# microsoft/NOTSOFAR1-Challenge

Measured on AMD Instinct MI355X. Metric: CSS real-time-factor (sep. audio sec/wall sec) on 7-ch 16 kHz, higher is better.
Workload: dtype f32 (float32 operands on v_mfma_f32_32x32x2_f32 in every Linear layer, attention product and transform: the reference's own operand precision; MVDR covariance / solve f64)

## Files before the change

include/css_mi355.h:

```cpp
#ifndef CSS_MI355_H
#define CSS_MI355_H

#include <stddef.h>
#include <stdint.h>

#ifdef __cplusplus
extern "C" {
#endif
#if defined(__GNUC__) || defined(__clang__)
#pragma GCC visibility push(default)
#endif

typedef struct css_ctx* css_handle_t;

typedef enum css_status {
    CSS_OK = 0,
    CSS_ERR_INVALID_ARG = -1,
    CSS_ERR_HIP = -2,
    CSS_ERR_ZERO_WEIGHT = -3,
    CSS_ERR_MASK_FLOOR = -4,
    CSS_ERR_SHAPE = -5,
    CSS_ERR_STATE = -6,
    CSS_ERR_NO_DEVICE = -7,
    CSS_ERR_WEIGHT_WINDOW = -8,
// ... 136 lines not shown
int css_run_enqueue(css_handle_t h, const float* pcm_host, int64_t n_samples, int32_t n_ch, const CssRunCfg* cfg,
                    float* wav_host, int64_t cap);
int css_set_queue_group(css_handle_t h, int max_sessions);
int css_wait(css_handle_t h);
int css_wait_sessions(css_handle_t h, int64_t n);
int css_run_device(css_handle_t h, const float* pcm_dev, int64_t n_samples, int32_t n_ch, const CssRunCfg* cfg,
                   float* wav_dev, int64_t wav_capacity_per_stream);
int css_run_pcm16(css_handle_t h, const int16_t* const* planes_host, int64_t n_samples, int32_t n_ch, const CssRunCfg* cfg,
                  int16_t* wav_pcm16_host, int64_t wav_capacity_per_stream, float* peaks_host);
int css_run_enqueue_pcm16(css_handle_t h, const int16_t* const* planes_host, int64_t n_samples, int32_t n_ch, const CssRunCfg* cfg,
                          int16_t* wav_pcm16_host, int64_t wav_capacity_per_stream, float* peaks_host);
int css_get_timings(css_handle_t h, CssTimings* out);
int css_set_profile(css_handle_t h, int enable);
typedef struct CssKernelStat { char name[32]; float ms; int32_t launches; } CssKernelStat;
int css_get_kernel_stats(css_handle_t h, CssKernelStat* out, int32_t cap, int32_t* count);
enum css_linear_mode { CSS_LINEAR_SPLIT_F16 = 0, CSS_LINEAR_EXACT_F32 = 1 };
int css_set_linear_mode(css_handle_t h, int mode);
int css_get_linear_mode(css_handle_t h);
int css_set_range_fallback(css_handle_t h, int enable);
int css_range_status(css_handle_t h, int64_t* fallbacks, int32_t* last_hit);
int css_check_range(css_handle_t h);
int css_linear_host(css_handle_t h, const float* x, const float* w, const float* bias, int32_t M, int32_t N, int32_t K,
                    int32_t kernel, int32_t layout, float* y);
int css_get_plan(css_handle_t h, CssPlan* out);

int css_begin(css_handle_t h, const float* pcm, int64_t n_samples, int32_t n_ch, const CssRunCfg* cfg, int pcm_is_device);
int css_begin_range(css_handle_t h, const float* pcm_host, int64_t n_samples, int32_t n_ch, const CssRunCfg* cfg,
                    int64_t s_lo, int64_t s_hi);
int css_upload_range(css_handle_t h, const float* pcm_host, int64_t s_lo, int64_t s_hi);
int css_stage_stft(css_handle_t h);
int css_stage_stft_range(css_handle_t h, int64_t t_lo, int64_t t_hi);
int css_stage_masknet(css_handle_t h, int64_t seg_lo, int64_t seg_hi);
int css_stage_mvdr(css_handle_t h, int64_t seg_lo, int64_t seg_hi);
int css_stage_pit_costs(css_handle_t h, int64_t b_lo, int64_t b_hi);
int css_stage_pit_scan(css_handle_t h);
int css_stage_stitch(css_handle_t h, int64_t t_lo, int64_t t_hi);
int css_stage_istft(css_handle_t h, int64_t t_lo, int64_t t_hi);
int css_stage_stitch_masks(css_handle_t h, int64_t t_lo, int64_t t_hi);
int css_stage_stitch_gate(css_handle_t h, int64_t t_lo, int64_t t_hi);
int css_stage_istft_partial(css_handle_t h, int64_t t_lo, int64_t t_hi, float* shard_dev, int64_t shard_ld);
int css_stage_synthesis(css_handle_t h, int64_t t_lo, int64_t t_hi);
int css_stage_seam_rows(css_handle_t h, int64_t t_lo, int64_t t_hi, float* rows_dev, int32_t write);
int css_stage_overlap_add(css_handle_t h, int64_t f_lo, int64_t f_hi, int64_t q_lo, int64_t q_hi, float* out_dev, int64_t out_ld,
                          int64_t out_q0);
int css_stage_join_shards(css_handle_t h, const float* gathered_dev, int32_t world, int64_t shard_ld, const int64_t* t_lo,
                          const int64_t* t_hi, float* out_dev, int64_t out_ld);
// ... 66 lines not shown
```

notsofar1-challenge_amd/_lib.py:

```python
from __future__ import annotations

import ctypes as C
import os
from typing import Optional

import numpy as np

_HERE = os.path.dirname(os.path.abspath(__file__))
LIB_PATH = os.environ.get("CSS_MI355_LIBRARY") or os.path.join(_HERE, "libcss_mi355.so")


class CssLibraryError(RuntimeError):
    pass


class CssError(RuntimeError):
    def __init__(self, code: int, text: str):
        super().__init__(f"css_mi355 error {code}: {text}")
        self.code = code
        self.text = text


CSS_OK, CSS_ERR_INVALID_ARG, CSS_ERR_HIP, CSS_ERR_ZERO_WEIGHT, CSS_ERR_MASK_FLOOR = 0, -1, -2, -3, -4
CSS_ERR_SHAPE, CSS_ERR_STATE, CSS_ERR_NO_DEVICE, CSS_ERR_WEIGHT_WINDOW, CSS_ERR_RANGE = -5, -6, -7, -8, -9
# ... 80 lines not shown
    "css_set_tuning": (C.c_int, [_P, C.c_int, C.c_int]),
    "css_set_queue_group": (C.c_int, [_P, C.c_int]),
    "css_host_alloc": (C.c_int, [C.c_size_t, C.POINTER(_P)]),
    "css_host_free": (C.c_int, [_P]),
    "css_plan": (C.c_int, [C.POINTER(CssModelDesc), C.POINTER(CssRunCfg), C.c_int64, C.POINTER(CssPlan)]),
    "css_make_run_cfg": (C.c_int, [C.POINTER(CssModelDesc), C.POINTER(CssCfgSeconds), C.c_int32, C.POINTER(CssRunCfg), _FP, C.c_int64]),
    "css_pit_scan": (C.c_int, [_P, C.c_int64, C.c_int32, _P]),
    "css_run": (C.c_int, [_P, _P, C.c_int64, C.c_int32, C.POINTER(CssRunCfg), _P, C.c_int64]),
    "css_run_enqueue": (C.c_int, [_P, _P, C.c_int64, C.c_int32, C.POINTER(CssRunCfg), _P, C.c_int64]),
    "css_wait": (C.c_int, [_P]),
    "css_wait_sessions": (C.c_int, [_P, C.c_int64]),
    "css_run_device": (C.c_int, [_P, _P, C.c_int64, C.c_int32, C.POINTER(CssRunCfg), _P, C.c_int64]),
    "css_run_pcm16": (C.c_int, [_P, _P, C.c_int64, C.c_int32, C.POINTER(CssRunCfg), _P, C.c_int64, _P]),
    "css_run_enqueue_pcm16": (C.c_int, [_P, _P, C.c_int64, C.c_int32, C.POINTER(CssRunCfg), _P, C.c_int64, _P]),
    "css_get_timings": (C.c_int, [_P, C.POINTER(CssTimings)]),
    "css_set_profile": (C.c_int, [_P, C.c_int]),
    "css_get_kernel_stats": (C.c_int, [_P, _P, C.c_int32, C.POINTER(C.c_int32)]),
    "css_set_linear_mode": (C.c_int, [_P, C.c_int]),
    "css_get_linear_mode": (C.c_int, [_P]),
    "css_set_range_fallback": (C.c_int, [_P, C.c_int]),
    "css_range_status": (C.c_int, [_P, C.POINTER(C.c_int64), C.POINTER(C.c_int32)]),
    "css_check_range": (C.c_int, [_P]),
    "css_linear_host": (C.c_int, [_P, _P, _P, _P, C.c_int32, C.c_int32, C.c_int32, C.c_int32, C.c_int32, _P]),
    "css_get_plan": (C.c_int, [_P, C.POINTER(CssPlan)]),
    "css_begin": (C.c_int, [_P, _P, C.c_int64, C.c_int32, C.POINTER(CssRunCfg), C.c_int]),
    "css_begin_range": (C.c_int, [_P, _P, C.c_int64, C.c_int32, C.POINTER(CssRunCfg), C.c_int64, C.c_int64]),
    "css_upload_range": (C.c_int, [_P, _P, C.c_int64, C.c_int64]),
    "css_stage_stft": (C.c_int, [_P]),
    "css_stage_stft_range": (C.c_int, [_P, C.c_int64, C.c_int64]),
    "css_stage_stitch_masks": (C.c_int, [_P, C.c_int64, C.c_int64]),
    "css_stage_stitch_gate": (C.c_int, [_P, C.c_int64, C.c_int64]),
    "css_stage_istft_partial": (C.c_int, [_P, C.c_int64, C.c_int64, _P, C.c_int64]),
    "css_stage_masknet": (C.c_int, [_P, C.c_int64, C.c_int64]),
    "css_stage_mvdr": (C.c_int, [_P, C.c_int64, C.c_int64]),
    "css_stage_pit_costs": (C.c_int, [_P, C.c_int64, C.c_int64]),
    "css_stage_pit_scan": (C.c_int, [_P]),
    "css_stage_stitch": (C.c_int, [_P, C.c_int64, C.c_int64]),
    "css_stage_istft": (C.c_int, [_P, C.c_int64, C.c_int64]),
    "css_stage_join_shards": (C.c_int, [_P, _P, C.c_int32, C.c_int64, _P, _P, _P, C.c_int64]),
    "css_stage_synthesis": (C.c_int, [_P, C.c_int64, C.c_int64]),
    "css_stage_seam_rows": (C.c_int, [_P, C.c_int64, C.c_int64, _P, C.c_int32]),
    "css_stage_overlap_add": (C.c_int, [_P, C.c_int64, C.c_int64, C.c_int64, C.c_int64, _P, C.c_int64, C.c_int64]),
    "css_sync": (C.c_int, [_P]),
    "css_stft_host": (C.c_int, [_P, _P, C.c_int64, C.c_int32, _P, C.c_int64]),
    "css_separate_host": (C.c_int, [_P, _P, C.c_int32, C.c_int32, _P]),
    "css_set_feature_options": (C.c_int, [_P, C.POINTER(CssFeatureCfg)]),
# ... 21 lines not shown
    "css_write_buffer": (C.c_int, [_P, C.c_int, _P, C.c_int64]),
    "css_buffer_devptr": (C.c_int, [_P, C.c_int, C.POINTER(_P)]),
}

_lib: Optional[C.CDLL] = None


def _share_hip_runtime_with_torch() -> None:
    import importlib.util
    try:
        spec = importlib.util.find_spec("torch")
    except (ImportError, ValueError):
        spec = None
    if spec is None or not spec.submodule_search_locations:
        return
    path = os.path.join(list(spec.submodule_search_locations)[0], "lib", "libamdhip64.so")
    if os.path.exists(path):
        try:
            C.CDLL(path, mode=C.RTLD_GLOBAL)
        except OSError:
            pass


def load() -> C.CDLL:
    global _lib
    if _lib is not None:
        return _lib
    if not os.path.exists(LIB_PATH):
        raise CssLibraryError(
            f"{LIB_PATH} not found: the HIP extension is not built. Run `python __graft_entry__.py` "
            f"(or `make -C notsofar1-challenge_amd/csrc`). There is no CPU fallback.")
    _share_hip_runtime_with_torch()
    try:
        lib = C.CDLL(LIB_PATH)
    except OSError as e:
        raise CssLibraryError(f"cannot load {LIB_PATH}: {e}") from e
    for name, (res, args) in SIGNATURES.items():
        fn = getattr(lib, name)
        fn.restype = res
        fn.argtypes = args
    _lib = lib
    return lib


def _np_ptr(a: np.ndarray):
    return a.ctypes.data_as(C.c_void_p)


def check(handle, rc: int):
    if rc != CSS_OK:
        text = load().css_last_error(handle).decode("utf-8", "replace")
        if rc == CSS_ERR_ZERO_WEIGHT:
            raise AssertionError(text or "zero weights found. check hop_size, segment_size or m0, m1")
        if rc == CSS_ERR_MASK_FLOOR:
            raise AssertionError(text)
        raise CssError(rc, text)


def make_desc(d) -> CssModelDesc:
    return CssModelDesc(*[int(getattr(d, n)) for n, _ in CssModelDesc._fields_])
# ... 228 lines not shown
    def set_range_fallback(self, enable: bool):
        check(self.h, self.lib.css_set_range_fallback(self.h, int(enable)))

    def range_status(self):
        n, last = C.c_int64(), C.c_int32()
        check(self.h, self.lib.css_range_status(self.h, C.byref(n), C.byref(last)))
        return int(n.value), bool(last.value)

    def check_range(self):
        check(self.h, self.lib.css_check_range(self.h))

    def linear(self, x: np.ndarray, w: np.ndarray, bias=None, kernel: int = 0, layout: int = 0) -> np.ndarray:
        x = np.ascontiguousarray(x, dtype=np.float32)
        w = np.ascontiguousarray(w, dtype=np.float32)
        m, k = x.shape
        n = w.shape[0]
        assert w.shape[1] == k
        b = None if bias is None else np.ascontiguousarray(bias, dtype=np.float32)
        y = np.empty((m, n), dtype=np.float32)
        check(self.h, self.lib.css_linear_host(self.h, _np_ptr(x), _np_ptr(w), _np_ptr(b) if b is not None else None,
                                               m, n, k, int(kernel), int(layout), _np_ptr(y)))
        return y

    def comm_init(self, unique_id: bytes, nranks: int, rank: int):
        assert len(unique_id) == COMM_ID_BYTES
        buf = C.create_string_buffer(bytes(unique_id), COMM_ID_BYTES)
        check(self.h, self.lib.css_comm_init(self.h, buf, int(nranks), int(rank)))

    def comm_destroy(self):
        check(self.h, self.lib.css_comm_destroy(self.h))

    def comm_info(self):
        n, r, d, v = C.c_int32(), C.c_int32(), C.c_int32(), C.c_int32()
        check(self.h, self.lib.css_comm_info(self.h, C.byref(n), C.byref(r), C.byref(d), C.byref(v)))
        return {"nranks": n.value, "rank": r.value, "device": d.value, "rccl_version_code": v.value}

    def comm_all_gather(self, send_ptr: int, recv_ptr: int, bytes_per_rank: int):
        check(self.h, self.lib.css_comm_all_gather(self.h, C.c_void_p(int(send_ptr)), C.c_void_p(int(recv_ptr)), int(bytes_per_rank)))

    def linear_mode(self):
        m = self.lib.css_get_linear_mode(self.h)
        if m < 0:
            check(self.h, m)
        return ("split_f16", "exact_f32")[m]

    def get_plan(self) -> CssPlan:
# ... 171 lines not shown
```

notsofar1-challenge_amd/csrc/api_core.hip:

```cpp
#include "api_ctx.hpp"

thread_local std::string g_create_error;

int fail(css_ctx* h, int code, const std::string& msg) {
    if (h) h->err = msg;
    else g_create_error = msg;
    return code;
}

int ensure(css_ctx* h, DevBuf& b, size_t bytes, bool zero) {
    if (bytes <= b.cap) return CSS_OK;
    if (b.p && h->queued) HIPCHK(h, hipDeviceSynchronize());
    if (b.p) HIPCHK(h, hipFree(b.p));
    b.p = nullptr;
    b.cap = 0;
    HIPCHK(h, hipMalloc(&b.p, bytes));
    b.cap = bytes;
    if (zero) HIPCHK(h, hipMemsetAsync(b.p, 0, bytes, h->stream));
    return CSS_OK;
}

int64_t bind_weights(const CssModelDesc& d, const float* base, Weights* w) {
    const int64_t D = d.attention_dim, FF = d.linear_units, Kp = round_up(d.in_features, 32);
    const int64_t dk = D / d.attention_heads, ks = d.kernel_size;
// ... 602 lines not shown
    return CSS_OK;
}

int css_range_status(css_handle_t h, int64_t* fallbacks, int32_t* last_hit) {
    if (!h) return CSS_ERR_INVALID_ARG;
    if (fallbacks) *fallbacks = h->range_fallbacks;
    if (last_hit) *last_hit = h->range_last;
    return CSS_OK;
}

int css_check_range(css_handle_t h) {
    int rc = check_session(h);
    if (rc) return rc;
    HIPCHK(h, hipSetDevice(h->device));
    HIPCHK(h, hipMemcpyAsync(h->range_flag_host, h->range_flag_dev, sizeof(unsigned int), hipMemcpyDeviceToHost, h->stream));
    HIPCHK(h, hipStreamSynchronize(h->stream));
    if (*h->range_flag_host && h->split)
        return fail(h, CSS_ERR_RANGE, "an operand of a Linear layer left the split-f16 range (|x| > 65504): use CSS_LINEAR_EXACT_F32");
    return CSS_OK;
}

int css_linear_host(css_handle_t h, const float* x, const float* w, const float* bias, int32_t M, int32_t N, int32_t K,
                    int32_t kernel, int32_t layout, float* y) {
    CSS_DRAIN(h);
    if (!h || !x || !w || !y || M < 1 || N < 1 || K < 32 || K % 32) return fail(h, CSS_ERR_INVALID_ARG, "bad argument (K must be a multiple of 32)");
    if (kernel < 0 || kernel > 2) return fail(h, CSS_ERR_INVALID_ARG, "kernel must be 0 (split, weights direct), 1 (split, LDS staged) or 2 (exact float32)");
    HIPCHK(h, hipSetDevice(h->device));
    const int Np = (N + 31) / 32 * 32;
    const size_t xf = (size_t)M * K, wf = (size_t)Np * K, yf = (size_t)M * N;
    int rc;
    if ((rc = ensure(h, h->stage, (2 * xf + 2 * wf + yf + (size_t)N + 256) * sizeof(float))) != CSS_OK) return rc;
    float* xd = (float*)h->stage.p;
    float* xs = xd + (xf + 15) / 16 * 16;
    float* wd = xs + (xf + 15) / 16 * 16;
    float* ws = wd + (wf + 15) / 16 * 16;
    float* yd = ws + (wf + 15) / 16 * 16;
    float* bd = yd + (yf + 15) / 16 * 16;
    HIPCHK(h, hipMemcpyAsync(xd, x, xf * sizeof(float), hipMemcpyHostToDevice, h->stream));
    HIPCHK(h, hipMemcpyAsync(wd, w, (size_t)N * K * sizeof(float), hipMemcpyHostToDevice, h->stream));
    if (bias) HIPCHK(h, hipMemcpyAsync(bd, bias, (size_t)N * sizeof(float), hipMemcpyHostToDevice, h->stream));
    GemmArgs g = linear(xd, K, wd, K, bias ? bd : nullptr, yd, N, M, N, K, ACT_NONE);
    if (kernel != 2) {
        launch_split_convert(xd, K, xs, M, K, K, h->stream);
        if (kernel == 0) launch_split_convert_tiled(wd, K, ws, N, K, h->stream);
        else launch_split_convert(wd, K, ws, N, K, K, h->stream);
        g.A = xs; g.B = ws; g.split_in = 1; g.b_tiled = kernel == 0;
        if (kernel == 0) g.tile_rows = layout; else g.layout = layout;
    } else {
        g.layout = layout;
    }
    launch_gemm(g, h->stream);
    HIPCHK(h, hipMemcpyAsync(y, yd, yf * sizeof(float), hipMemcpyDeviceToHost, h->stream));
    HIPCHK(h, hipStreamSynchronize(h->stream));
    HIPCHK(h, hipGetLastError());
    return CSS_OK;
}

int css_host_alloc(size_t bytes, void** out) {
    if (!out) return CSS_ERR_INVALID_ARG;
    *out = nullptr;
    return hipHostMalloc(out, bytes ? bytes : 1, hipHostMallocDefault) == hipSuccess ? CSS_OK : CSS_ERR_HIP;
}

int css_host_free(void* p) { return (!p || hipHostFree(p) == hipSuccess) ? CSS_OK : CSS_ERR_HIP; }

int css_set_linear_mode(css_handle_t h, int mode) {
    CSS_DRAIN(h);
    if (!h || (mode != CSS_LINEAR_SPLIT_F16 && mode != CSS_LINEAR_EXACT_F32)) return fail(h, CSS_ERR_INVALID_ARG, "unknown linear mode");
    const bool split = mode == CSS_LINEAR_SPLIT_F16;
    if (split == h->split) return CSS_OK;
    if (split && stream_open_count(h)) return fail(h, CSS_ERR_STATE, "a stream is open: streams run in CSS_LINEAR_EXACT_F32 only");
    if (split && !h->split_ok) return fail(h, CSS_ERR_RANGE, "a weight of this model lies outside the split-f16 operand range (|w| > 65504)");
// ... 353 lines not shown
```

notsofar1-challenge_amd/csrc/gemm_f32.hip:

```cpp
#include <algorithm>
#include <type_traits>

#include "gemm_common.hpp"

namespace css {

namespace {

constexpr int F_BK = 16;
constexpr int F_LD = 20;
constexpr int F_BUF = (128 + BN) * F_LD;
constexpr int F_PATCH_LD = 36;

typedef float f32x4 __attribute__((ext_vector_type(4)));

__device__ __forceinline__ float epi_value(float acc, float bn, float bm, int act, bool has_res, float rv, float alpha) {
    float v = acc + bn + bm;
    if (act == ACT_RELU) v = fmaxf(v, 0.f);
    else if (act == ACT_SIGMOID) v = sigmoidf_(v);
    if (has_res) v = rv + alpha * v;
    return v;
}

template <int TM, bool BD, bool FAST>
__device__ __forceinline__ void f32_tile(const GemmArgs& g, const float* __restrict__ A, const float* __restrict__ B,
                                         float* __restrict__ C, const int m0, const int n0, float* __restrict__ lds) {
// ... 14 lines not shown
#ifndef F32_PROBE
#define F32_PROBE 0
#endif
#ifndef F32_FAST_EPILOGUE
#define F32_FAST_EPILOGUE 1
#endif
#ifndef F32_SPREAD
#define F32_SPREAD 1
#endif
#ifndef F32_TRANSPOSED
#define F32_TRANSPOSED 0
#endif
#ifndef F32_STORE_GUARD
#define F32_STORE_GUARD 1
#endif
#if F32_STORE_GUARD
#define F32_AFTER_STORE(o) asm volatile("s_nop 0" : : "v"(o));
#else
#define F32_AFTER_STORE(o)
#endif
#ifndef F32_DMA
#define F32_DMA 0
#endif
#if F32_DMA
    constexpr int D_BUF = (128 + BN) * 16;
    const int dseg = ((tid & 3) ^ ((tid >> 4) & 3)) * 4;
    const int dvoA = (int)(((int64_t)(m0 + srow) * g.lda + dseg) * 4), dvoB = (int)(((int64_t)(n0 + srow) * g.ldb + dseg) * 4);
    const bool a1_wave = (BM % 64 == 0) || w < (BM % 64) / 16;
    typedef __attribute__((address_space(3))) void lds_void;
#define F32_GLOAD(k0, buf)                                                                                       \
    _Pragma("unroll") for (int i = 0; i < NPA; ++i) {                                                            \
        if (i + 1 < NPA || a1_wave)                                                                              \
            __builtin_amdgcn_raw_ptr_buffer_load_lds(rsA, (lds_void*)(lds + (buf) * D_BUF + (i * 64 + 16 * w) * 16), 16, dvoA, (k0) * 4 + i * passA, 0, 0); \
    }                                                                                                            \
    _Pragma("unroll") for (int i = 0; i < 2; ++i)                                                                \
        __builtin_amdgcn_raw_ptr_buffer_load_lds(rsB, (lds_void*)(lds + (buf) * D_BUF + (128 + i * 64 + 16 * w) * 16), 16, dvoB, (k0) * 4 + i * passB, 0, 0);
#define F32_LSTORE(buf) __builtin_amdgcn_s_waitcnt(0x0F70);
#define F32_GLOAD1(k0, j)
#undef F32_SPREAD
#define F32_SPREAD 0
#else
    f32x4 ra[NPA], rb[2];
    f32x4 wc[2], wn[2];
    const int vw = (int)((((int64_t)(n0 / 32 + w) * (g.K / 8)) * 64 + lane) * 16);
#define F32_GLOAD(k0, buf)                                                                                       \
    _Pragma("unroll") for (int i = 0; i < NPA; ++i) {                                                            \
        if (i + 1 < NPA || a1_on) ra[i] = __builtin_bit_cast(f32x4, __builtin_amdgcn_raw_buffer_load_b128(rsA, voA, (k0) * 4 + i * passA, 0)); \
    }                                                                                                            \
    if constexpr (!BD) {                                                                                         \
        _Pragma("unroll") for (int i = 0; i < 2; ++i)                                                            \
            rb[i] = __builtin_bit_cast(f32x4, __builtin_amdgcn_raw_buffer_load_b128(rsB, voB, (k0) * 4 + i * passB, 0)); \
    } else {                                                                                                     \
        wn[0] = __builtin_bit_cast(f32x4, __builtin_amdgcn_raw_buffer_load_b128(rsB, vw, ((k0) / 8) * 1024, 0)); \
        wn[1] = __builtin_bit_cast(f32x4, __builtin_amdgcn_raw_buffer_load_b128(rsB, vw, ((k0) / 8 + 1) * 1024, 0)); \
    }
#define F32_GLOAD1(k0, j)                                                                                        \
    {                                                                                                            \
        if ((j) < NPA) {                                                                                         \
            if ((j) + 1 < NPA || a1_on) ra[(j) < NPA ? (j) : 0] = __builtin_bit_cast(f32x4, __builtin_amdgcn_raw_buffer_load_b128(rsA, voA, (k0) * 4 + (j) * passA, 0)); \
        } else if ((j) < NPA + 2) {                                                                              \
            if constexpr (!BD) rb[(j) - NPA] = __builtin_bit_cast(f32x4, __builtin_amdgcn_raw_buffer_load_b128(rsB, voB, (k0) * 4 + ((j) - NPA) * passB, 0)); \
            else wn[(j) - NPA] = __builtin_bit_cast(f32x4, __builtin_amdgcn_raw_buffer_load_b128(rsB, vw, ((k0) / 8 + (j) - NPA) * 1024, 0)); \
        }                                                                                                        \
    }
#define F32_LSTORE(buf)                                                                                          \
    {                                                                                                            \
        float* as_ = lds + (buf) * F_BUF + srow * F_LD + sk;                                                     \
        _Pragma("unroll") for (int i = 0; i < NPA; ++i) {                                                        \
            if (i + 1 < NPA || a1_on) *reinterpret_cast<f32x4*>(as_ + i * 64 * F_LD) = ra[i];                    \
        }                                                                                                        \
        if constexpr (!BD) {                                                                                     \
            _Pragma("unroll") for (int i = 0; i < 2; ++i) *reinterpret_cast<f32x4*>(as_ + (128 + i * 64) * F_LD) = rb[i]; \
        }                                                                                                        \
    }
#endif
    f32x16 acc[TM];
#pragma unroll
    for (int i = 0; i < TM; ++i) acc[i] = f32x16{0};
    const int nk = g.K / F_BK;
#if F32_PROBE
    const unsigned long long t_in_ = (w == 0) ? __builtin_readcyclecounter() : 0;
#endif
    F32_GLOAD(0, 0)
    F32_LSTORE(0)
    if constexpr (BD) { wc[0] = wn[0]; wc[1] = wn[1]; }
    __syncthreads();
#if F32_DMA
    constexpr int S_BUF = D_BUF, S_LD = 16;
    const int sw4 = ((c >> 2) & 3) * 4;
    const int aoff = c * 16, boff = (128 + 32 * w + c) * 16;
#define F32_SLOT(ch) (((8 * (ch) + 4 * h)) ^ sw4)
#else
    constexpr int S_BUF = F_BUF, S_LD = F_LD;
    const int aoff = c * F_LD + 4 * h, boff = (128 + 32 * w + c) * F_LD + 4 * h;
#define F32_SLOT(ch) (8 * (ch))
#endif
    const float* __restrict__ bias = g.bias;
    const float* __restrict__ res = g.residual;
    const int act = g.act;
    const bool bias_m = bias && g.bias_along_m, bias_n = bias && !g.bias_along_m, has_res = res != nullptr;
    const int64_t ldc = g.ldc, ldr = g.ldr;
    const float alpha = g.alpha;
    const bool wide = FAST || ((ldc % 4 == 0) && (N % 4 == 0) && ((reinterpret_cast<uintptr_t>(C) & 15) == 0) &&
                               (!has_res || ((ldr % 4 == 0) && ((reinterpret_cast<uintptr_t>(res) & 15) == 0))));
    constexpr bool fast = FAST;
    const __amdgpu_buffer_rsrc_t rsC = __builtin_amdgcn_make_buffer_rsrc(C, 0, fast ? (int)((int64_t)M * ldc * 4) : 0, 0x00020000);
    const __amdgpu_buffer_rsrc_t rsR = __builtin_amdgcn_make_buffer_rsrc(const_cast<float*>(res), 0, (fast && has_res) ? (int)((int64_t)M * ldr * 4) : 0, 0x00020000);
    f32x4 rv[2][4];
// ... 13 lines not shown
    };
#endif
    auto prefetch = [&](int i, int slot, int lane_) {
        const int n_ = n0 + 32 * w + (lane_ & 7) * 4;
#pragma unroll
        for (int j = 0; j < 4; ++j) {
            const int m = m0 + 32 * i + (lane_ >> 3) + 8 * j;
            const int mc = m < M ? m : M - 1;
            rv[slot][j] = f32x4{0.f, 0.f, 0.f, 0.f};
            if (has_res && n_ < N) {
                if (wide) {
                    rv[slot][j] = *reinterpret_cast<const f32x4*>(res + (int64_t)mc * ldr + n_);
                } else {
#pragma unroll
                    for (int e = 0; e < 4; ++e) rv[slot][j][e] = res[(int64_t)mc * ldr + (n_ + e < N ? n_ + e : N - 1)];
                }
            }
        }
    };
#ifndef F32_ABLATE
#define F32_ABLATE 0
#endif
    f32x4 abl_a = {1.f, 2.f, 3.f, (float)lane}, abl_b = {0.5f, 0.25f, (float)w, 1.f};
#define F32_COMPUTE(buf)                                                                                         \
    {                                                                                                            \
        const float* as = lds + (buf) * S_BUF + aoff;                                                            \
        const float* bs = lds + (buf) * S_BUF + boff;                                                            \
        _Pragma("unroll") for (int ch = 0; ch < 2; ++ch) {                                                       \
            f32x4 b = abl_b;                                                                                     \
            if constexpr (BD) b = wc[ch];                                                                        \
            else if (!(F32_ABLATE & 4)) b = *reinterpret_cast<const f32x4*>(bs + F32_SLOT(ch));                  \
            f32x4 a[TM];                                                                                         \
            _Pragma("unroll") for (int i = 0; i < TM; ++i) {                                                     \
                a[i] = abl_a;                                                                                    \
                if (!(F32_ABLATE & 4)) a[i] = *reinterpret_cast<const f32x4*>(as + i * 32 * S_LD + F32_SLOT(ch)); \
            }                                                                                                    \
            __builtin_amdgcn_sched_barrier(0);                                                                   \
            _Pragma("unroll") for (int e = 0; e < 4; ++e) {                                                      \
                if (F32_SPREAD && spread_k0 >= 0 && !(e & 1)) { F32_GLOAD1(spread_k0, ch * 2 + (e >> 1)) __builtin_amdgcn_sched_barrier(0); } \
                _Pragma("unroll") for (int i = 0; i < TM; ++i) {                                                 \
                    if (F32_ABLATE & 8) asm volatile("v_mfma_f32_32x32x2_f32 %0, %1, %2, %0" : "+a"(acc[i]) : "v"(a[i][e]), "v"(b[e])); \
                    else if (F32_TRANSPOSED) acc[i] = __builtin_amdgcn_mfma_f32_32x32x2f32(b[e], a[i][e], acc[i], 0, 0, 0); \
                    else acc[i] = __builtin_amdgcn_mfma_f32_32x32x2f32(a[i][e], b[e], acc[i], 0, 0, 0);          \
                }                                                                                                \
                if (F32_SPREAD && spread_k0 >= 0) __builtin_amdgcn_sched_barrier(0);                             \
            }                                                                                                    \
            __builtin_amdgcn_sched_barrier(0);                                                                   \
        }                                                                                                        \
    }
#if F32_PROBE
    const bool probe = w == 0 && g.narrow_epilogue == 77 && g.range_flag;
    unsigned long long pc_ = 0, pl_ = 0, pb_ = 0, pt_ = 0;
    const unsigned long long t_loop_ = probe ? __builtin_readcyclecounter() : 0;
#define F32_CLK(var) if (probe) var = __builtin_readcyclecounter();
#else
#define F32_CLK(var)
#endif
    int spread_k0 = -1;
    for (int kt = 0; kt + 1 < nk; ++kt) {
#if F32_PROBE
        unsigned long long t0_ = 0, t1_ = 0, t2_ = 0, t3_ = 0;
#endif
        F32_CLK(t0_)
        if (F32_SPREAD) spread_k0 = (kt + 1) * F_BK;
        else if (!(F32_ABLATE & 2)) { F32_GLOAD((kt + 1) * F_BK, (kt + 1) & 1) }
        __builtin_amdgcn_sched_barrier(0);
        F32_COMPUTE(kt & 1)
        F32_CLK(t1_)
        if (!(F32_ABLATE & 2)) { F32_LSTORE((kt + 1) & 1) }
        if constexpr (BD) { wc[0] = wn[0]; wc[1] = wn[1]; }
        F32_CLK(t2_)
        if (!(F32_ABLATE & 1)) __syncthreads();
        F32_CLK(t3_)
#if F32_PROBE
        pc_ += t1_ - t0_; pl_ += t2_ - t1_; pb_ += t3_ - t2_; pt_ += 1;
#endif
    }
#if F32_PROBE
    if (probe && lane == 0) {
        unsigned long long* pr = reinterpret_cast<unsigned long long*>(g.range_flag) + 4096 + 4 * blockIdx.x;
        atomicAdd(pr + 0, pc_); atomicAdd(pr + 1, pl_); atomicAdd(pr + 2, pb_); atomicAdd(pr + 3, pt_);
        atomicAdd(pr + 4096 + 0, t_loop_ - t_in_);
        atomicAdd(pr + 4096 + 1, 1ull);
    }
    const unsigned long long t_out_ = probe ? __builtin_readcyclecounter() : 0;
#define F32_EPILOGUE_PROBE                                                                                       \
    if (probe && lane == 0) {                                                                                    \
        unsigned long long* pr = reinterpret_cast<unsigned long long*>(g.range_flag) + 4096 + 4 * blockIdx.x;    \
        atomicAdd(pr + 4096 + 2, __builtin_readcyclecounter() - t_out_);        \
    }
#else
#define F32_EPILOGUE_PROBE
#endif
#undef F32_CLK
    {
        int lane_ = lane;
        asm volatile("" : "+v"(lane_));
        if (fast) { if (has_res) prefetch_fast(0, 0, lane_); }
        else prefetch(0, 0, lane_);
    }
    spread_k0 = -1;
    F32_COMPUTE((nk - 1) & 1)
    __syncthreads();
#undef F32_COMPUTE
#undef F32_SLOT
#undef F32_GLOAD
#undef F32_GLOAD1
#undef F32_LSTORE

    int lane_e = lane;
    asm volatile("" : "+v"(lane_e));
    float* patch = lds + w * (32 * F_PATCH_LD);
    const int col4 = (lane_e & 7) * 4, n = n0 + 32 * w + col4, erow = lane_e >> 3;
    const bool col_ok = n < N;
    float bn[4] = {0.f, 0.f, 0.f, 0.f};
    if (bias_n) {
#pragma unroll
        for (int e = 0; e < 4; ++e) bn[e] = bias[n + e < N ? n + e : N - 1];
    }
#if F32_TRANSPOSED
    if (fast) {
        const int ce = lane_e & 31, he = lane_e >> 5, nw = n0 + 32 * w + 4 * he;
        const int voC = (int)((((int64_t)m0 + ce) * ldc + nw) * 4);
        const bool relu = act == ACT_RELU;
        f32x4 bq[4];
// ... 85 lines not shown
            const int row = erow + 8 * j, m = m0 + 32 * i + row;
            const f32x4 v = *reinterpret_cast<const f32x4*>(patch + row * F_PATCH_LD + col4);
            if (m >= M || !col_ok) continue;
            float* dst = C + (int64_t)m * ldc + n;
            const float bm = bias_m ? bias[m] : 0.f;
            f32x4 o;
#pragma unroll
            for (int e = 0; e < 4; ++e) o[e] = epi_value(v[e], bn[e], bm, act, has_res, rv[i & 1][j][e], alpha);
            if (wide) {
                *reinterpret_cast<f32x4*>(dst) = o;
            } else {
#pragma unroll
                for (int e = 0; e < 4; ++e)
                    if (n + e < N) dst[e] = o[e];
            }
        }
    }
    F32_EPILOGUE_PROBE
#undef F32_EPILOGUE_PROBE
}

}

struct F32Plan {
    int u, tiles_n, ncu, max_tm; int64_t U;
#if F32_TOOLS
    unsigned long long* dbg;
#endif
};

template <bool BD, bool FAST>
__global__ __launch_bounds__(256, 4) void gemm_f32_kernel(GemmArgs g, F32Plan p) {
    __shared__ __attribute__((aligned(16))) float lds[2 * F_BUF];
    const int b = blockIdx.x, v = b % p.ncu, j = b / p.ncu;
    const int64_t lo = p.U * v / p.ncu, hi = p.U * (v + 1) / p.ncu;
    int64_t pos = lo + (hi - lo) * j / 4;
    const int64_t end = lo + (hi - lo) * (j + 1) / 4;
    int want = std::min(1 + (b + j) % 4, p.max_tm);
    bool first = true;
#if F32_TOOLS
    if (p.dbg && threadIdx.x == 0) {
        p.dbg[4 * b + 0] = wall_clock64();
        p.dbg[4 * b + 2] = ((unsigned long long)__builtin_amdgcn_s_getreg(63508) << 32) | (unsigned)__builtin_amdgcn_s_getreg(63492);
        p.dbg[4 * b + 3] = __builtin_readcyclecounter();
    }
#endif
    const int64_t panel0 = pos / p.u;
    int r = (int)(pos - panel0 * p.u);
    int bz = (int)(panel0 / p.tiles_n), tn = (int)(panel0 - (int64_t)bz * p.tiles_n);
    while (pos < end) {
        const int tm = (int)std::min<int64_t>(std::min<int64_t>(want, end - pos), p.u - r);
        const float* A = g.A + (int64_t)bz * g.strideA;
        const float* B = g.B + (int64_t)bz * g.strideB;
        float* C = g.C + (int64_t)bz * g.strideC;
        if (!first) __syncthreads();
        first = false;
        switch (tm) {
            case 1: f32_tile<1, BD, FAST>(g, A, B, C, 32 * r, tn * BN, lds); break;
            case 2: f32_tile<2, BD, FAST>(g, A, B, C, 32 * r, tn * BN, lds); break;
            case 3: f32_tile<3, BD, FAST>(g, A, B, C, 32 * r, tn * BN, lds); break;
            default: f32_tile<4, BD, FAST>(g, A, B, C, 32 * r, tn * BN, lds); break;
        }
        pos += tm;
        want = p.max_tm;
        r += tm;
        if (r == p.u) {
            r = 0;
            if (++tn == p.tiles_n) { tn = 0; ++bz; }
        }
    }
#if F32_TOOLS
    if (p.dbg && threadIdx.x == 0) { p.dbg[4 * b + 1] = wall_clock64(); p.dbg[4 * b + 3] = __builtin_readcyclecounter() - p.dbg[4 * b + 3]; }
#endif
}

static bool f32_fast_epilogue(const GemmArgs& g) {
    const int64_t lim = (int64_t)1 << 31;
    const bool has_res = g.residual != nullptr;
    const bool wide = (g.ldc % 4 == 0) && (g.N % 4 == 0) && ((reinterpret_cast<uintptr_t>(g.C) & 15) == 0) &&
                      (g.batch == 1 || g.strideC % 4 == 0) &&
                      (!has_res || ((g.ldr % 4 == 0) && ((reinterpret_cast<uintptr_t>(g.residual) & 15) == 0)));
    return F32_FAST_EPILOGUE && wide && !(g.bias && g.bias_along_m) && (g.N % BN == 0) && g.act != ACT_SIGMOID &&
           (int64_t)g.M * g.ldc * 4 < lim && (!has_res || (int64_t)g.M * g.ldr * 4 < lim);
}

bool launch_gemm_f32(const GemmArgs& g, hipStream_t s, int forced_tm) {
    if (g.M <= 0 || g.N <= 0 || g.batch <= 0) return true;
    if (g.K <= 0 || g.K % F_BK) return false;
    const int64_t lim = (int64_t)1 << 31;
    if ((((int64_t)g.M + 128) * g.lda + g.K) * 4 >= lim || (((int64_t)g.N + 128) * g.ldb + g.K) * 4 >= lim) return false;
    if (g.b_frag32 && (g.N % 32 || g.K % 16 || g.batch != 1 || ((int64_t)g.N * g.K * 4 >= lim))) return false;
    if ((g.lda % 4) || (!g.b_frag32 && (g.ldb % 4)) || (reinterpret_cast<uintptr_t>(g.A) & 15) || (reinterpret_cast<uintptr_t>(g.B) & 15)) return false;
    constexpr int NCU = 256;
    F32Plan p;
    p.u = (g.M + 31) / 32;
    p.tiles_n = (g.N + BN - 1) / BN;
    p.ncu = NCU;
    p.max_tm = (forced_tm >= 1 && forced_tm <= 4) ? forced_tm : 4;
    p.U = (int64_t)p.u * p.tiles_n * g.batch;
#if F32_TOOLS
    p.dbg = g.narrow_epilogue == 77 ? reinterpret_cast<unsigned long long*>(g.range_flag) : nullptr;
#endif
    const bool fast = f32_fast_epilogue(g);
    void (*kern)(GemmArgs, F32Plan) = g.b_frag32 ? (fast ? gemm_f32_kernel<true, true> : gemm_f32_kernel<true, false>)
                                                 : (fast ? gemm_f32_kernel<false, true> : gemm_f32_kernel<false, false>);
    hipLaunchKernelGGL(kern, dim3(4 * NCU), dim3(256), 0, s, g, p);
    return true;
}


__global__ void f32_fragments_kernel(const float* __restrict__ src, int64_t ld_src, float* __restrict__ dst, int N, int K) {
    const int64_t idx = (int64_t)blockIdx.x * blockDim.x + threadIdx.x;
    const int64_t total = (int64_t)(N / 32) * (K / 8) * 64;
    if (idx >= total) return;
    const int lane = (int)(idx & 63);
    const int64_t t = idx >> 6;
    const int kc = (int)(t % (K / 8)), j = (int)(t / (K / 8));
    const float* p = src + (int64_t)(32 * j + (lane & 31)) * ld_src + 8 * kc + 4 * (lane >> 5);
    reinterpret_cast<float4*>(dst)[idx] = make_float4(p[0], p[1], p[2], p[3]);
}
void launch_f32_fragments(const float* src, int64_t ld_src, float* dst, int N, int K, hipStream_t s) {
    const int64_t total = (int64_t)(N / 32) * (K / 8) * 64;
    if (total <= 0) return;
    hipLaunchKernelGGL(f32_fragments_kernel, dim3((unsigned)((total + 255) / 256)), dim3(256), 0, s, src, ld_src, dst, N, K);
}

}
// ... 1 lines not shown
```

Measured before the change: 7109.

## Deepen f32 GEMM prefetch to two register sets and rebalance tile heights

The f32 MFMA GEMM gets double-buffered register prefetch sets (PD=2) for tiles with TM<=2 in the non-DMA path, so global loads are issued two k-steps ahead and their latency is hidden behind compute. The persistent tile walk moves into a shared header and changes how row tiles are split: it avoids leaving 1- or 2-row remainder tiles in a panel by choosing the first height so the rest splits into 3- or 4-row tiles. A test-only linear_host_ex entry point adds residual, ReLU and fragment-weight options for validation. The extra prefetch set raises register pressure, which could reduce occupancy under the 256x4 launch bounds.

```diff
diff --git a/include/css_mi355.h b/include/css_mi355.h
--- a/include/css_mi355.h
+++ b/include/css_mi355.h
@@ -182,6 +182,8 @@
 int css_check_range(css_handle_t h);
 int css_linear_host(css_handle_t h, const float* x, const float* w, const float* bias, int32_t M, int32_t N, int32_t K,
                     int32_t kernel, int32_t layout, float* y);
+int css_linear_host_ex(css_handle_t h, const float* x, const float* w, const float* bias, const float* residual, float alpha,
+                       int32_t act, int32_t frag_weights, int32_t M, int32_t N, int32_t K, int32_t kernel, int32_t layout, float* y);
 int css_get_plan(css_handle_t h, CssPlan* out);
 
 int css_begin(css_handle_t h, const float* pcm, int64_t n_samples, int32_t n_ch, const CssRunCfg* cfg, int pcm_is_device);
diff --git a/notsofar1-challenge_amd/_lib.py b/notsofar1-challenge_amd/_lib.py
--- a/notsofar1-challenge_amd/_lib.py
+++ b/notsofar1-challenge_amd/_lib.py
@@ -126,6 +126,8 @@
     "css_range_status": (C.c_int, [_P, C.POINTER(C.c_int64), C.POINTER(C.c_int32)]),
     "css_check_range": (C.c_int, [_P]),
     "css_linear_host": (C.c_int, [_P, _P, _P, _P, C.c_int32, C.c_int32, C.c_int32, C.c_int32, C.c_int32, _P]),
+    "css_linear_host_ex": (C.c_int, [_P, _P, _P, _P, _P, C.c_float, C.c_int32, C.c_int32, C.c_int32, C.c_int32, C.c_int32, C.c_int32,
+                                     C.c_int32, _P]),
     "css_get_plan": (C.c_int, [_P, C.POINTER(CssPlan)]),
     "css_begin": (C.c_int, [_P, _P, C.c_int64, C.c_int32, C.POINTER(CssRunCfg), C.c_int]),
     "css_begin_range": (C.c_int, [_P, _P, C.c_int64, C.c_int32, C.POINTER(CssRunCfg), C.c_int64, C.c_int64]),
@@ -193,6 +195,9 @@
             pass
 
 
+TEST_ONLY = frozenset({"css_linear_host_ex"})
+
+
 def load() -> C.CDLL:
     global _lib
     if _lib is not None:
@@ -207,6 +212,8 @@
     except OSError as e:
         raise CssLibraryError(f"cannot load {LIB_PATH}: {e}") from e
     for name, (res, args) in SIGNATURES.items():
+        if name in TEST_ONLY and not hasattr(lib, name):
+            continue
         fn = getattr(lib, name)
         fn.restype = res
         fn.argtypes = args
@@ -481,6 +488,22 @@
                                                m, n, k, int(kernel), int(layout), _np_ptr(y)))
         return y
 
+    def linear_ex(self, x: np.ndarray, w: np.ndarray, bias=None, residual=None, alpha: float = 1.0, relu: bool = False,
+                  frag_weights: bool = False, kernel: int = 2, layout: int = 0) -> np.ndarray:
+        x = np.ascontiguousarray(x, dtype=np.float32)
+        w = np.ascontiguousarray(w, dtype=np.float32)
+        m, k = x.shape
+        n = w.shape[0]
+        assert w.shape[1] == k
+        b = None if bias is None else np.ascontiguousarray(bias, dtype=np.float32)
+        r = None if residual is None else np.ascontiguousarray(residual, dtype=np.float32)
+        assert r is None or r.shape == (m, n)
+        y = np.empty((m, n), dtype=np.float32)
+        check(self.h, self.lib.css_linear_host_ex(self.h, _np_ptr(x), _np_ptr(w), _np_ptr(b) if b is not None else None,
+                                                  _np_ptr(r) if r is not None else None, float(alpha), int(bool(relu)),
+                                                  int(bool(frag_weights)), m, n, k, int(kernel), int(layout), _np_ptr(y)))
+        return y
+
     def comm_init(self, unique_id: bytes, nranks: int, rank: int):
         assert len(unique_id) == COMM_ID_BYTES
         buf = C.create_string_buffer(bytes(unique_id), COMM_ID_BYTES)
diff --git a/notsofar1-challenge_amd/csrc/api_core.hip b/notsofar1-challenge_amd/csrc/api_core.hip
--- a/notsofar1-challenge_amd/csrc/api_core.hip
+++ b/notsofar1-challenge_amd/csrc/api_core.hip
@@ -648,24 +648,34 @@
 
 int css_linear_host(css_handle_t h, const float* x, const float* w, const float* bias, int32_t M, int32_t N, int32_t K,
                     int32_t kernel, int32_t layout, float* y) {
+    return css_linear_host_ex(h, x, w, bias, nullptr, 1.f, 0, 0, M, N, K, kernel, layout, y);
+}
+
+int css_linear_host_ex(css_handle_t h, const float* x, const float* w, const float* bias, const float* residual, float alpha,
+                       int32_t act, int32_t frag_weights, int32_t M, int32_t N, int32_t K, int32_t kernel, int32_t layout, float* y) {
     CSS_DRAIN(h);
     if (!h || !x || !w || !y || M < 1 || N < 1 || K < 32 || K % 32) return fail(h, CSS_ERR_INVALID_ARG, "bad argument (K must be a multiple of 32)");
     if (kernel < 0 || kernel > 2) return fail(h, CSS_ERR_INVALID_ARG, "kernel must be 0 (split, weights direct), 1 (split, LDS staged) or 2 (exact float32)");
+    if (act != ACT_NONE && act != ACT_RELU) return fail(h, CSS_ERR_INVALID_ARG, "act must be 0 (none) or 1 (ReLU)");
+    if (frag_weights && (kernel != 2 || N % 32)) return fail(h, CSS_ERR_INVALID_ARG, "fragment-ordered weights: the exact float32 kernel and N % 32 == 0 only");
     HIPCHK(h, hipSetDevice(h->device));
     const int Np = (N + 31) / 32 * 32;
     const size_t xf = (size_t)M * K, wf = (size_t)Np * K, yf = (size_t)M * N;
     int rc;
-    if ((rc = ensure(h, h->stage, (2 * xf + 2 * wf + yf + (size_t)N + 256) * sizeof(float))) != CSS_OK) return rc;
+    if ((rc = ensure(h, h->stage, (2 * xf + 2 * wf + 2 * yf + (size_t)N + 256) * sizeof(float))) != CSS_OK) return rc;
     float* xd = (float*)h->stage.p;
     float* xs = xd + (xf + 15) / 16 * 16;
     float* wd = xs + (xf + 15) / 16 * 16;
     float* ws = wd + (wf + 15) / 16 * 16;
     float* yd = ws + (wf + 15) / 16 * 16;
-    float* bd = yd + (yf + 15) / 16 * 16;
+    float* rd = yd + (yf + 15) / 16 * 16;
+    float* bd = rd + (yf + 15) / 16 * 16;
     HIPCHK(h, hipMemcpyAsync(xd, x, xf * sizeof(float), hipMemcpyHostToDevice, h->stream));
     HIPCHK(h, hipMemcpyAsync(wd, w, (size_t)N * K * sizeof(float), hipMemcpyHostToDevice, h->stream));
     if (bias) HIPCHK(h, hipMemcpyAsync(bd, bias, (size_t)N * sizeof(float), hipMemcpyHostToDevice, h->stream));
-    GemmArgs g = linear(xd, K, wd, K, bias ? bd : nullptr, yd, N, M, N, K, ACT_NONE);
+    if (residual) HIPCHK(h, hipMemcpyAsync(rd, residual, yf * sizeof(float), hipMemcpyHostToDevice, h->stream));
+    GemmArgs g = linear(xd, K, wd, K, bias ? bd : nullptr, yd, N, M, N, K, act);
+    if (residual) { g.residual = rd; g.ldr = N; g.alpha = alpha; }
     if (kernel != 2) {
         launch_split_convert(xd, K, xs, M, K, K, h->stream);
         if (kernel == 0) launch_split_convert_tiled(wd, K, ws, N, K, h->stream);
@@ -674,6 +684,10 @@
         if (kernel == 0) g.tile_rows = layout; else g.layout = layout;
     } else {
         g.layout = layout;
+        if (frag_weights) {
+            launch_f32_fragments(wd, K, ws, N, K, h->stream);
+            g.B = ws; g.b_frag32 = 1; g.B_rows = wd;
+        }
     }
     launch_gemm(g, h->stream);
     HIPCHK(h, hipMemcpyAsync(y, yd, yf * sizeof(float), hipMemcpyDeviceToHost, h->stream));
diff --git a/notsofar1-challenge_amd/csrc/gemm_f32.hip b/notsofar1-challenge_amd/csrc/gemm_f32.hip
--- a/notsofar1-challenge_amd/csrc/gemm_f32.hip
+++ b/notsofar1-challenge_amd/csrc/gemm_f32.hip
@@ -2,6 +2,7 @@
 #include <type_traits>
 
 #include "gemm_common.hpp"
+#include "gemm_f32_walk.hpp"
 
 namespace css {
 
@@ -62,55 +63,56 @@
 #ifndef F32_DMA
 #define F32_DMA 0
 #endif
+    constexpr int PD = (F32_DMA || TM > 2) ? 1 : 2;
 #if F32_DMA
     constexpr int D_BUF = (128 + BN) * 16;
     const int dseg = ((tid & 3) ^ ((tid >> 4) & 3)) * 4;
     const int dvoA = (int)(((int64_t)(m0 + srow) * g.lda + dseg) * 4), dvoB = (int)(((int64_t)(n0 + srow) * g.ldb + dseg) * 4);
     const bool a1_wave = (BM % 64 == 0) || w < (BM % 64) / 16;
     typedef __attribute__((address_space(3))) void lds_void;
-#define F32_GLOAD(k0, buf)                                                                                       \
+#define F32_GLOAD(k0, set)                                                                                       \
     _Pragma("unroll") for (int i = 0; i < NPA; ++i) {                                                            \
         if (i + 1 < NPA || a1_wave)                                                                              \
-            __builtin_amdgcn_raw_ptr_buffer_load_lds(rsA, (lds_void*)(lds + (buf) * D_BUF + (i * 64 + 16 * w) * 16), 16, dvoA, (k0) * 4 + i * passA, 0, 0); \
+            __builtin_amdgcn_raw_ptr_buffer_load_lds(rsA, (lds_void*)(lds + (((k0) / F_BK) & 1) * D_BUF + (i * 64 + 16 * w) * 16), 16, dvoA, (k0) * 4 + i * passA, 0, 0); \
     }                                                                                                            \
     _Pragma("unroll") for (int i = 0; i < 2; ++i)                                                                \
-        __builtin_amdgcn_raw_ptr_buffer_load_lds(rsB, (lds_void*)(lds + (buf) * D_BUF + (128 + i * 64 + 16 * w) * 16), 16, dvoB, (k0) * 4 + i * passB, 0, 0);
-#define F32_LSTORE(buf) __builtin_amdgcn_s_waitcnt(0x0F70);
-#define F32_GLOAD1(k0, j)
+        __builtin_amdgcn_raw_ptr_buffer_load_lds(rsB, (lds_void*)(lds + (((k0) / F_BK) & 1) * D_BUF + (128 + i * 64 + 16 * w) * 16), 16, dvoB, (k0) * 4 + i * passB, 0, 0);
+#define F32_LSTORE(buf, set) __builtin_amdgcn_s_waitcnt(0x0F70);
+#define F32_GLOAD1(k0, j, set)
 #undef F32_SPREAD
 #define F32_SPREAD 0
 #else
-    f32x4 ra[NPA], rb[2];
-    f32x4 wc[2], wn[2];
+    f32x4 ra[PD][NPA], rb[PD][2];
+    f32x4 wc[2], wn[PD][2];
     const int vw = (int)((((int64_t)(n0 / 32 + w) * (g.K / 8)) * 64 + lane) * 16);
-#define F32_GLOAD(k0, buf)                                                                                       \
+#define F32_GLOAD(k0, set)                                                                                       \
     _Pragma("unroll") for (int i = 0; i < NPA; ++i) {                                                            \
-        if (i + 1 < NPA || a1_on) ra[i] = __builtin_bit_cast(f32x4, __builtin_amdgcn_raw_buffer_load_b128(rsA, voA, (k0) * 4 + i * passA, 0)); \
+        if (i + 1 < NPA || a1_on) ra[set][i] = __builtin_bit_cast(f32x4, __builtin_amdgcn_raw_buffer_load_b128(rsA, voA, (k0) * 4 + i * passA, 0)); \
     }                                                                                                            \
     if constexpr (!BD) {                                                                                         \
         _Pragma("unroll") for (int i = 0; i < 2; ++i)                                                            \
-            rb[i] = __builtin_bit_cast(f32x4, __builtin_amdgcn_raw_buffer_load_b128(rsB, voB, (k0) * 4 + i * passB, 0)); \
+            rb[set][i] = __builtin_bit_cast(f32x4, __builtin_amdgcn_raw_buffer_load_b128(rsB, voB, (k0) * 4 + i * passB, 0)); \
     } else {                                                                                                     \
-        wn[0] = __builtin_bit_cast(f32x4, __builtin_amdgcn_raw_buffer_load_b128(rsB, vw, ((k0) / 8) * 1024, 0)); \
-        wn[1] = __builtin_bit_cast(f32x4, __builtin_amdgcn_raw_buffer_load_b128(rsB, vw, ((k0) / 8 + 1) * 1024, 0)); \
-    }
-#define F32_GLOAD1(k0, j)                                                                                        \
+        wn[set][0] = __builtin_bit_cast(f32x4, __builtin_amdgcn_raw_buffer_load_b128(rsB, vw, ((k0) / 8) * 1024, 0)); \
+        wn[set][1] = __builtin_bit_cast(f32x4, __builtin_amdgcn_raw_buffer_load_b128(rsB, vw, ((k0) / 8 + 1) * 1024, 0)); \
+    }
+#define F32_GLOAD1(k0, j, set)                                                                                   \
     {                                                                                                            \
         if ((j) < NPA) {                                                                                         \
-            if ((j) + 1 < NPA || a1_on) ra[(j) < NPA ? (j) : 0] = __builtin_bit_cast(f32x4, __builtin_amdgcn_raw_buffer_load_b128(rsA, voA, (k0) * 4 + (j) * passA, 0)); \
+            if ((j) + 1 < NPA || a1_on) ra[set][(j) < NPA ? (j) : 0] = __builtin_bit_cast(f32x4, __builtin_amdgcn_raw_buffer_load_b128(rsA, voA, (k0) * 4 + (j) * passA, 0)); \
         } else if ((j) < NPA + 2) {                                                                              \
-            if constexpr (!BD) rb[(j) - NPA] = __builtin_bit_cast(f32x4, __builtin_amdgcn_raw_buffer_load_b128(rsB, voB, (k0) * 4 + ((j) - NPA) * passB, 0)); \
-            else wn[(j) - NPA] = __builtin_bit_cast(f32x4, __builtin_amdgcn_raw_buffer_load_b128(rsB, vw, ((k0) / 8 + (j) - NPA) * 1024, 0)); \
+            if constexpr (!BD) rb[set][(j) - NPA] = __builtin_bit_cast(f32x4, __builtin_amdgcn_raw_buffer_load_b128(rsB, voB, (k0) * 4 + ((j) - NPA) * passB, 0)); \
+            else wn[set][(j) - NPA] = __builtin_bit_cast(f32x4, __builtin_amdgcn_raw_buffer_load_b128(rsB, vw, ((k0) / 8 + (j) - NPA) * 1024, 0)); \
         }                                                                                                        \
     }
-#define F32_LSTORE(buf)                                                                                          \
+#define F32_LSTORE(buf, set)                                                                                     \
     {                                                                                                            \
         float* as_ = lds + (buf) * F_BUF + srow * F_LD + sk;                                                     \
         _Pragma("unroll") for (int i = 0; i < NPA; ++i) {                                                        \
-            if (i + 1 < NPA || a1_on) *reinterpret_cast<f32x4*>(as_ + i * 64 * F_LD) = ra[i];                    \
+            if (i + 1 < NPA || a1_on) *reinterpret_cast<f32x4*>(as_ + i * 64 * F_LD) = ra[set][i];               \
         }                                                                                                        \
         if constexpr (!BD) {                                                                                     \
-            _Pragma("unroll") for (int i = 0; i < 2; ++i) *reinterpret_cast<f32x4*>(as_ + (128 + i * 64) * F_LD) = rb[i]; \
+            _Pragma("unroll") for (int i = 0; i < 2; ++i) *reinterpret_cast<f32x4*>(as_ + (128 + i * 64) * F_LD) = rb[set][i]; \
         }                                                                                                        \
     }
 #endif
@@ -122,8 +124,9 @@
     const unsigned long long t_in_ = (w == 0) ? __builtin_readcyclecounter() : 0;
 #endif
     F32_GLOAD(0, 0)
-    F32_LSTORE(0)
-    if constexpr (BD) { wc[0] = wn[0]; wc[1] = wn[1]; }
+    if (PD == 2 && nk > 1) { F32_GLOAD(F_BK, PD - 1) }
+    F32_LSTORE(0, 0)
+    if constexpr (BD) { wc[0] = wn[0][0]; wc[1] = wn[0][1]; }
     __syncthreads();
 #if F32_DMA
     constexpr int S_BUF = D_BUF, S_LD = 16;
@@ -183,7 +186,7 @@
 #define F32_ABLATE 0
 #endif
     f32x4 abl_a = {1.f, 2.f, 3.f, (float)lane}, abl_b = {0.5f, 0.25f, (float)w, 1.f};
-#define F32_COMPUTE(buf)                                                                                         \
+#define F32_COMPUTE(buf, set)                                                                                      \
     {                                                                                                            \
         const float* as = lds + (buf) * S_BUF + aoff;                                                            \
         const float* bs = lds + (buf) * S_BUF + boff;                                                            \
@@ -198,7 +201,7 @@
             }                                                                                                    \
             __builtin_amdgcn_sched_barrier(0);                                                                   \
             _Pragma("unroll") for (int e = 0; e < 4; ++e) {                                                      \
-                if (F32_SPREAD && spread_k0 >= 0 && !(e & 1)) { F32_GLOAD1(spread_k0, ch * 2 + (e >> 1)) __builtin_amdgcn_sched_barrier(0); } \
+                if (F32_SPREAD && spread_k0 >= 0 && !(e & 1)) { F32_GLOAD1(spread_k0, ch * 2 + (e >> 1), set) __builtin_amdgcn_sched_barrier(0); } \
                 _Pragma("unroll") for (int i = 0; i < TM; ++i) {                                                 \
                     if (F32_ABLATE & 8) asm volatile("v_mfma_f32_32x32x2_f32 %0, %1, %2, %0" : "+a"(acc[i]) : "v"(a[i][e]), "v"(b[e])); \
                     else if (F32_TRANSPOSED) acc[i] = __builtin_amdgcn_mfma_f32_32x32x2f32(b[e], a[i][e], acc[i], 0, 0, 0); \
@@ -218,24 +221,29 @@
 #define F32_CLK(var)
 #endif
     int spread_k0 = -1;
-    for (int kt = 0; kt + 1 < nk; ++kt) {
+    for (int kt0 = 0; kt0 + 1 < nk; kt0 += PD) {
+#pragma unroll
+    for (int q = 0; q < PD; ++q) {
+        const int kt = kt0 + q;
+        if (q > 0 && kt + 1 >= nk) break;
 #if F32_PROBE
         unsigned long long t0_ = 0, t1_ = 0, t2_ = 0, t3_ = 0;
 #endif
         F32_CLK(t0_)
-        if (F32_SPREAD) spread_k0 = (kt + 1) * F_BK;
-        else if (!(F32_ABLATE & 2)) { F32_GLOAD((kt + 1) * F_BK, (kt + 1) & 1) }
+        if (F32_SPREAD) spread_k0 = (kt + PD) * F_BK;
+        else if (!(F32_ABLATE & 2)) { F32_GLOAD((kt + PD) * F_BK, q) }
         __builtin_amdgcn_sched_barrier(0);
-        F32_COMPUTE(kt & 1)
+        F32_COMPUTE(kt & 1, q)
         F32_CLK(t1_)
-        if (!(F32_ABLATE & 2)) { F32_LSTORE((kt + 1) & 1) }
-        if constexpr (BD) { wc[0] = wn[0]; wc[1] = wn[1]; }
+        if (!(F32_ABLATE & 2)) { F32_LSTORE((kt + 1) & 1, (q + 1) % PD) }
+        if constexpr (BD) { wc[0] = wn[(q + 1) % PD][0]; wc[1] = wn[(q + 1) % PD][1]; }
         F32_CLK(t2_)
         if (!(F32_ABLATE & 1)) __syncthreads();
         F32_CLK(t3_)
 #if F32_PROBE
         pc_ += t1_ - t0_; pl_ += t2_ - t1_; pb_ += t3_ - t2_; pt_ += 1;
 #endif
+    }
     }
 #if F32_PROBE
     if (probe && lane == 0) {
@@ -261,7 +269,7 @@
         else prefetch(0, 0, lane_);
     }
     spread_k0 = -1;
-    F32_COMPUTE((nk - 1) & 1)
+    F32_COMPUTE((nk - 1) & 1, 0)
     __syncthreads();
 #undef F32_COMPUTE
 #undef F32_SLOT
@@ -393,21 +401,19 @@
 
 }
 
-struct F32Plan {
-    int u, tiles_n, ncu, max_tm; int64_t U;
 #if F32_TOOLS
+struct F32Args : F32Plan {
     unsigned long long* dbg;
-#endif
 };
+#else
+typedef F32Plan F32Args;
+#endif
 
 template <bool BD, bool FAST>
-__global__ __launch_bounds__(256, 4) void gemm_f32_kernel(GemmArgs g, F32Plan p) {
+__global__ __launch_bounds__(256, 4) void gemm_f32_kernel(GemmArgs g, F32Args p) {
     __shared__ __attribute__((aligned(16))) float lds[2 * F_BUF];
-    const int b = blockIdx.x, v = b % p.ncu, j = b / p.ncu;
-    const int64_t lo = p.U * v / p.ncu, hi = p.U * (v + 1) / p.ncu;
-    int64_t pos = lo + (hi - lo) * j / 4;
-    const int64_t end = lo + (hi - lo) * (j + 1) / 4;
-    int want = std::min(1 + (b + j) % 4, p.max_tm);
+    const int b = blockIdx.x;
+    F32Walk walk = f32_walk_begin(p, b);
     bool first = true;
 #if F32_TOOLS
     if (p.dbg && threadIdx.x == 0) {
@@ -416,28 +422,18 @@
         p.dbg[4 * b + 3] = __builtin_readcyclecounter();
     }
 #endif
-    const int64_t panel0 = pos / p.u;
-    int r = (int)(pos - panel0 * p.u);
-    int bz = (int)(panel0 / p.tiles_n), tn = (int)(panel0 - (int64_t)bz * p.tiles_n);
-    while (pos < end) {
-        const int tm = (int)std::min<int64_t>(std::min<int64_t>(want, end - pos), p.u - r);
-        const float* A = g.A + (int64_t)bz * g.strideA;
-        const float* B = g.B + (int64_t)bz * g.strideB;
-        float* C = g.C + (int64_t)bz * g.strideC;
+    F32Tile t;
+    while (f32_walk_next(p, walk, t)) {
+        const float* A = g.A + (int64_t)t.bz * g.strideA;
+        const float* B = g.B + (int64_t)t.bz * g.strideB;
+        float* C = g.C + (int64_t)t.bz * g.strideC;
         if (!first) __syncthreads();
         first = false;
-        switch (tm) {
-            case 1: f32_tile<1, BD, FAST>(g, A, B, C, 32 * r, tn * BN, lds); break;
-            case 2: f32_tile<2, BD, FAST>(g, A, B, C, 32 * r, tn * BN, lds); break;
-            case 3: f32_tile<3, BD, FAST>(g, A, B, C, 32 * r, tn * BN, lds); break;
-            default: f32_tile<4, BD, FAST>(g, A, B, C, 32 * r, tn * BN, lds); break;
-        }
-        pos += tm;
-        want = p.max_tm;
-        r += tm;
-        if (r == p.u) {
-            r = 0;
-            if (++tn == p.tiles_n) { tn = 0; ++bz; }
+        switch (t.tm) {
+            case 1: f32_tile<1, BD, FAST>(g, A, B, C, 32 * t.r, t.tn * BN, lds); break;
+            case 2: f32_tile<2, BD, FAST>(g, A, B, C, 32 * t.r, t.tn * BN, lds); break;
+            case 3: f32_tile<3, BD, FAST>(g, A, B, C, 32 * t.r, t.tn * BN, lds); break;
+            default: f32_tile<4, BD, FAST>(g, A, B, C, 32 * t.r, t.tn * BN, lds); break;
         }
     }
 #if F32_TOOLS
@@ -463,7 +459,7 @@
     if (g.b_frag32 && (g.N % 32 || g.K % 16 || g.batch != 1 || ((int64_t)g.N * g.K * 4 >= lim))) return false;
     if ((g.lda % 4) || (!g.b_frag32 && (g.ldb % 4)) || (reinterpret_cast<uintptr_t>(g.A) & 15) || (reinterpret_cast<uintptr_t>(g.B) & 15)) return false;
     constexpr int NCU = 256;
-    F32Plan p;
+    F32Args p;
     p.u = (g.M + 31) / 32;
     p.tiles_n = (g.N + BN - 1) / BN;
     p.ncu = NCU;
@@ -473,7 +469,7 @@
     p.dbg = g.narrow_epilogue == 77 ? reinterpret_cast<unsigned long long*>(g.range_flag) : nullptr;
 #endif
     const bool fast = f32_fast_epilogue(g);
-    void (*kern)(GemmArgs, F32Plan) = g.b_frag32 ? (fast ? gemm_f32_kernel<true, true> : gemm_f32_kernel<true, false>)
+    void (*kern)(GemmArgs, F32Args) = g.b_frag32 ? (fast ? gemm_f32_kernel<true, true> : gemm_f32_kernel<true, false>)
                                                  : (fast ? gemm_f32_kernel<false, true> : gemm_f32_kernel<false, false>);
     hipLaunchKernelGGL(kern, dim3(4 * NCU), dim3(256), 0, s, g, p);
     return true;
diff --git a/notsofar1-challenge_amd/csrc/gemm_f32_walk.hpp b/notsofar1-challenge_amd/csrc/gemm_f32_walk.hpp
--- /dev/null
+++ b/notsofar1-challenge_amd/csrc/gemm_f32_walk.hpp
@@ -0,0 +1,84 @@
+#pragma once
+#include <stdint.h>
+
+#if defined(__HIPCC__) || defined(__CUDACC__)
+#define F32_WALK_FN __host__ __device__ inline
+#else
+#define F32_WALK_FN inline
+#endif
+
+namespace css {
+
+struct F32Plan {
+    int u, tiles_n, ncu, max_tm;
+    int64_t U;
+};
+
+struct F32Walk {
+    int64_t pos, end;
+    int r, tn, bz;
+    int left;
+    int want;
+};
+
+struct F32Tile {
+    int tm;
+    int r, tn, bz;
+};
+
+F32_WALK_FN int f32_first_height(int n, int want, int max_tm) {
+    if (want > max_tm) want = max_tm;
+    if (max_tm < 4) return want < n ? want : n;
+    if (n <= 3) return n;
+    int f = want;
+    for (int k = 0; k < 4; ++k) {
+        f = (want - 1 + k) % 4 + 1;
+        const int rem = n - f;
+        if (rem == 0 || rem >= 3) break;
+    }
+    return f;
+}
+
+F32_WALK_FN int f32_next_height(int left, int max_tm) {
+    if (max_tm < 4) return max_tm < left ? max_tm : left;
+    return (left & 3) ? (left & 3) : 4;
+}
+
+F32_WALK_FN F32Walk f32_walk_begin(const F32Plan& p, int b) {
+    const int v = b % p.ncu, j = b / p.ncu;
+    const int64_t lo = p.U * v / p.ncu, hi = p.U * (v + 1) / p.ncu;
+    F32Walk w;
+    w.pos = lo + (hi - lo) * j / 4;
+    w.end = lo + (hi - lo) * (j + 1) / 4;
+    const int64_t panel0 = w.pos / p.u;
+    w.r = (int)(w.pos - panel0 * p.u);
+    w.bz = (int)(panel0 / p.tiles_n);
+    w.tn = (int)(panel0 - (int64_t)w.bz * p.tiles_n);
+    w.left = 0;
+    w.want = 1 + (b + j) % 4;
+    return w;
+}
+
+F32_WALK_FN bool f32_walk_next(const F32Plan& p, F32Walk& w, F32Tile& t) {
+    if (w.pos >= w.end) return false;
+    if (w.left == 0) {
+        const int64_t piece = w.end - w.pos;
+        const int panel = p.u - w.r;
+        w.left = piece < panel ? (int)piece : panel;
+        t.tm = f32_first_height(w.left, w.want, p.max_tm);
+        w.want = p.max_tm;
+    } else {
+        t.tm = f32_next_height(w.left, p.max_tm);
+    }
+    t.r = w.r; t.tn = w.tn; t.bz = w.bz;
+    w.pos += t.tm;
+    w.left -= t.tm;
+    w.r += t.tm;
+    if (w.r == p.u) {
+        w.r = 0;
+        if (++w.tn == p.tiles_n) { w.tn = 0; ++w.bz; }
+    }
+    return true;
+}
+
+}
```

Result: no change. 7145, median of 6 (+0.5%).
